# jskvrna/MonoSOWA

Measured on AMD Instinct MI355X. Metric: MonoDETR training img/s (KITTI 1280x384), higher is better.
Workload: dtype f32; 1 GPU; MonoDETR resnet50 KITTI 1280x384, fwd+criterion+bwd+AdamW step, per-GPU batch 16, synthetic images + random pseudo-labels; global_batch=16, per_gpu_batch=16, parallelism=dp1, accumulation_micro_steps=1, mixed_cameras=False, queries=550, tuned=True

## Files before the change

### include/monosowa_pointwise.h

```cpp
#ifndef MONOSOWA_POINTWISE_H_
#define MONOSOWA_POINTWISE_H_
#ifdef __cplusplus
extern "C" {
#endif

int mono_set_deterministic(int on);

int mono_bias_act_f32(float *y, const float *bias, const float *residual, long long rows, int C, int relu, void *stream);
int mono_bias_relu_maxpool_nhwc_f32(const float *y, const float *bias, float *out, int N, int H, int W, int C, void *stream);
int mono_conv1x1_tail_f32(const float *x, const float *b_in, const float *w, const float *b_out, const float *res, float *y,
                          long long M, int K, int N, void *stream);
int mono_conv1x1_tail_ds_f32(const float *x, const float *b_in, const float *w, const float *x0, const float *wd, const float *b_out,
                             float *y, long long M, int K, int N, void *stream);
int mono_conv1x1_head_f32(const float *x, const float *w, const float *b_out, float *y, long long M, int K, int N, void *stream);

int mono_relu_grad_f32(const float *grad_out, const float *y, float *grad_in, long long n, void *stream);
int mono_relu_grad_scale_f32(const float *grad_out, const float *y, const float *scale, float *grad_in, long long n, int C, void *stream);

int mono_bias_relu_mask_f32(float *y, const float *bias, const float *residual, unsigned char *mask, long long rows, int C,
                            void *stream);
int mono_relu_grad_mask_f32(const float *grad_a, const float *grad_b, const unsigned char *mask, float *grad_in, long long n,
                            void *stream);
int mono_relu_grad_mask3_f32(const float *grad_a, const float *grad_b, const float *grad_c, const unsigned char *mask, float *grad_in,
                             long long n, void *stream);
// ... 40 lines not shown
int mono_grad_guard_f32(const void *const *tables, const int *n_chunks, int n_groups, float max_norm, int skip_nonfinite,
                        double *partials, void *record, void *stream);
int mono_adamw_step_guarded_f32(const void *table, int n_chunks, double beta1, double beta2, double eps, double step_size,
                                const void *record, void *stream);

int mono_grad_accumulate_f32(const void *table, int n_chunks, void *stream);

int mono_ema_update_f32(const void *table, int n_chunks, float w, const void *record, void *stream);

int mono_step_stats_f32(const void *const *tables, const int *n_chunks, const int *const *groups, int n_tables, int n_groups,
                        const void *record, double *partials, double *out, void *stream);

long long mono_linear_wgrad_workspace(int R, int M, int N);
int mono_linear_wgrad_f32(const float *dy, long long ldy, const float *x, long long ldx, float *dw, float *db, float *ws, int R, int M,
                          int N, void *stream);

int mono_colsum_any_blocks(long long rows);
int mono_colsum_any_f32(const float *g, float *out, float *partials, long long rows, int C, void *stream);

int mono_sum_slices_f32(const float *x, float *out, int n, long long C, void *stream);

int mono_reduce_blocks(long long rows);

int mono_dropout_add_layernorm_bwd_f32(const float *gy, const float *s, const float *mean, const float *rstd,
                                       const float *gamma, float *gx, float *gz, float *ggamma_gbeta, float *partials,
                                       long long rows, int C, float p, unsigned long long seed, void *stream);

int mono_colsum_f32(const float *g, float *out, float *partials, long long rows, int C, void *stream);
int mono_colsum_strided_f32(const float *g, float *out, float *partials, int batch, long long rows, long long batch_stride,
                            int C, void *stream);
// ... 111 lines not shown
```

### monosowa_amd/csrc/pointwise.hip

```cpp
#include <hip/hip_runtime.h>

#include "relu_nan.h"
#include "groupnorm.hip"
#include "matched_losses.hip"
#include "ddn_loss.hip"
#include "head_tail.hip"
#include "lsap_device.hip"
#include "conv1x1_fused.hip"
#include "small_wgrad.hip"
#include <stdint.h>
#include <algorithm>

namespace mono {

template <bool RELU, bool RES>
__global__ __launch_bounds__(256) void bias_act_kernel(float *__restrict__ y, const float *__restrict__ bias,
                                                       const float *__restrict__ residual, long long n_vec, int c_vec) {
  const long long stride = (long long)gridDim.x * blockDim.x;
  for (long long i = (long long)blockIdx.x * blockDim.x + threadIdx.x; i < n_vec; i += stride) {
    float4 v = reinterpret_cast<float4 *>(y)[i];
    const float4 b = reinterpret_cast<const float4 *>(bias)[i % c_vec];
    v.x += b.x; v.y += b.y; v.z += b.z; v.w += b.w;
    if (RES) {
      const float4 r = reinterpret_cast<const float4 *>(residual)[i];
// ... 1081 lines not shown
  if (rows <= 0 || C <= 0 || C % 4 || C > 1024) return -2;
  hipStream_t st = (hipStream_t)stream_;
  if (rows <= mono::kColsumStripRows && C <= 384) {
    mono::colsum_strip_kernel<<<(C / 4 + 3) / 4, 1024, 0, st>>>(g, out, rows, C);
    return (int)hipGetLastError();
  }
  const int grid = mono_reduce_blocks(rows);
  const int rpb = (int)((rows + grid - 1) / grid + 63) / 64 * 64;
  if (C <= 256) mono::colsum_kernel<1><<<grid, 256, 0, st>>>(g, partials, rows, C, rpb, rows, 0);
  else if (C <= 512) mono::colsum_kernel<2><<<grid, 256, 0, st>>>(g, partials, rows, C, rpb, rows, 0);
  else mono::colsum_kernel<4><<<grid, 256, 0, st>>>(g, partials, rows, C, rpb, rows, 0);
  mono::partial_sum_kernel<<<(C / 4 + 63) / 64, 1024, 0, st>>>(partials, out, grid, C);
  return (int)hipGetLastError();
}

long long mono_linear_wgrad_workspace(int R, int M, int N) {
  if (R < 64 || R >= (1 << 24) || M <= 0 || N <= 0 || M % 64 || N % 64 || M > 4096 || N > 4096) return 0;
  return (long long)mono::linear_wgrad_splits(R, M, N) * ((long long)M * N + M);
}
int mono_linear_wgrad_f32(const float *dy, long long ldy, const float *x, long long ldx, float *dw, float *db, float *ws, int R, int M,
                          int N, void *stream_) {
  if (!dy || !x || !dw || !ws) return -1;
  if (!mono_linear_wgrad_workspace(R, M, N) || ldy < M || ldx < N || ldy % 4 || ldx % 4 || ((size_t)dy | (size_t)x | (size_t)dw | (size_t)ws) % 16 ||
      (db && (size_t)db % 16))
    return -2;
  hipStream_t st = (hipStream_t)stream_;
  const int S = mono::linear_wgrad_splits(R, M, N);
  const int rows_per_split = ((R + S - 1) / S + mono::kWgStageRows - 1) / mono::kWgStageRows * mono::kWgStageRows;
  const int tiles = (M / 64) * (N / 64);
  mono::linear_wgrad_partial_kernel<<<tiles * S, 256, 0, st>>>(dy, ldy, x, ldx, ws, R, M, N, S, rows_per_split);
  const long long MN = (long long)M * N;
  mono::linear_wgrad_reduce_kernel<<<(int)(((MN + M) / 4 + 255) / 256), 256, 0, st>>>(ws, dw, db, MN, M, S);
  return (int)hipGetLastError();
}

int mono_colsum_any_blocks(long long rows) {
  const long long b = (rows + 127) / 128;
  return (int)(b < 1 ? 1 : (b > 512 ? 512 : b));
}
int mono_colsum_any_f32(const float *g, float *out, float *partials, long long rows, int C, void *stream_) {
  if (!g || !out || !partials) return -1;
  if (rows <= 0 || C <= 0 || C > 1024) return -2;
  const int grid = mono_colsum_any_blocks(rows);
  const int rpb = (int)((rows + grid - 1) / grid);
  hipStream_t st = (hipStream_t)stream_;
  mono::colsum_scalar_kernel<<<grid, 256, 0, st>>>(g, partials, rows, C, rpb);
  mono::partial_sum_scalar_kernel<<<(C + 255) / 256, 256, 0, st>>>(partials, out, grid, C);
  return (int)hipGetLastError();
// ... 421 lines not shown
```

### monosowa_amd/csrc/small_wgrad.hip

```cpp
#pragma once
#include <hip/hip_runtime.h>

namespace mono {

typedef float wg_f32x16 __attribute__((ext_vector_type(16)));
#ifndef MONO_WGRAD_WORKGROUPS
#define MONO_WGRAD_WORKGROUPS 256
#endif
constexpr int kWgPairs = 8;
constexpr int kWgStageRows = 2 * kWgPairs;
constexpr int kWgSlots = 3;

inline int linear_wgrad_splits(int R, int M, int N) {
  const int tiles = (M / 64) * (N / 64);
  int S = ((MONO_WGRAD_WORKGROUPS + tiles - 1) / tiles + 7) / 8 * 8;
  while (S > 8 && R / S < 64) S -= 8;
  return S;
}

__global__ __launch_bounds__(256) void linear_wgrad_partial_kernel(const float *__restrict__ dy, long long ldy,
                                                                   const float *__restrict__ x, long long ldx, float *__restrict__ ws,
                                                                   int R, int M, int N, int S, int rows_per_split) {
  __shared__ float ring[kWgSlots][2][kWgStageRows * 64];
  const int s = blockIdx.x % S, tile = blockIdx.x / S;
  const int n_tiles = N / 64, tm = tile / n_tiles, tn = tile % n_tiles;
  const int lane = threadIdx.x & 63, wave = __builtin_amdgcn_readfirstlane(threadIdx.x >> 6), c = lane & 31, h = lane >> 5;
  const int wm = wave >> 1, wn = wave & 1;
  const int m0 = tm * 64 + wm * 32, n0 = tn * 64 + wn * 32;
  const int k_begin = s * rows_per_split, k_end = min(R, k_begin + rows_per_split);
  const int n_stages = k_end > k_begin ? (k_end - k_begin) / kWgStageRows : 0;
  wg_f32x16 acc0 = {0.f, 0.f, 0.f, 0.f, 0.f, 0.f, 0.f, 0.f, 0.f, 0.f, 0.f, 0.f, 0.f, 0.f, 0.f, 0.f}, acc1 = acc0;
  float bsum = 0.f;
  const int src_row = 4 * ((2 * wave) & 3) + 2 * (lane >> 5) + ((lane >> 3) & 1), src_col = 32 * ((lane >> 4) & 1) + 4 * (lane & 7);
  const float *gsrc = wave < 2 ? dy + (long long)(k_begin + src_row) * ldy + tm * 64 + src_col
                               : x + (long long)(k_begin + src_row) * ldx + tn * 64 + src_col;
  const long long g_ld = wave < 2 ? ldy : ldx;
  float *const lds_dst = &ring[0][wave >> 1][((2 * wave) & 3) * 256 + 4 * lane];
  constexpr int kSlotFloats = 2 * kWgStageRows * 64;
  const float *const al = &ring[0][0][wm * 64 + lane], *const bl = &ring[0][1][wn * 64 + lane];
  float4 g0a, g0b, g1a, g1b, g2a, g2b, g3a, g3b;
  float a0[kWgPairs], b0[kWgPairs], a1[kWgPairs], b1[kWgPairs];
#define WG_GLOAD(GA, GB, STAGE)                                                                                      \
  {                                                                                                                  \
    const float *p_ = gsrc + (long long)min((STAGE), n_stages - 1) * kWgStageRows * g_ld;              \
    GA = *reinterpret_cast<const float4 *>(p_); GB = *reinterpret_cast<const float4 *>(p_ + 4 * g_ld);               \
  }
#define WG_LWRITE(GA, GB, STAGE)                                                                                     \
  {                                                                                                                  \
    float *d_ = lds_dst + ((STAGE) % kWgSlots) * kSlotFloats;                                                        \
    *reinterpret_cast<float4 *>(d_) = GA; *reinterpret_cast<float4 *>(d_ + 256) = GB;                                \
  }
#define WG_STAGE(AC, BC, AN, BN, GA, GB, I)                                                                          \
  {                                                                                                                  \
    float *d_ = lds_dst + (((I) + 2) % kWgSlots) * kSlotFloats;                                                      \
    _Pragma("unroll") for (int u = 0; u < kWgPairs / 2; ++u) {                                                       \
      if (u & 1) acc1 = __builtin_amdgcn_mfma_f32_32x32x2f32(AC[u], BC[u], acc1, 0, 0, 0);                           \
      else acc0 = __builtin_amdgcn_mfma_f32_32x32x2f32(AC[u], BC[u], acc0, 0, 0, 0);                                 \
      bsum += AC[u];                                                                                                 \
      if (u < 2) {                           \
        __builtin_amdgcn_sched_barrier(0);                                                                           \
        *reinterpret_cast<float4 *>(d_ + 256 * u) = u ? GB : GA;                                                     \
        __builtin_amdgcn_sched_barrier(0);                                                                           \
      }                                                                                                              \
    }                                                                                                                \
    __builtin_amdgcn_sched_barrier(0);                                                                               \
    asm volatile("s_waitcnt lgkmcnt(0)" ::: "memory");                                                               \
    __builtin_amdgcn_s_barrier();                                                                                    \
    __builtin_amdgcn_sched_barrier(0);                                                                               \
    WG_GLOAD(GA, GB, (I) + 6)                                                                                        \
    __builtin_amdgcn_sched_barrier(0);                                                                               \
    const float *an_ = al + (((I) + 1) % kWgSlots) * kSlotFloats, *bn_ = bl + (((I) + 1) % kWgSlots) * kSlotFloats;  \
    _Pragma("unroll") for (int u = kWgPairs / 2; u < kWgPairs; ++u) {                                                \
      if (u & 1) acc1 = __builtin_amdgcn_mfma_f32_32x32x2f32(AC[u], BC[u], acc1, 0, 0, 0);                           \
      else acc0 = __builtin_amdgcn_mfma_f32_32x32x2f32(AC[u], BC[u], acc0, 0, 0, 0);                                 \
      bsum += AC[u];                                                                                                 \
      const int v = (u - kWgPairs / 2) * 2;                                                                          \
      AN[v] = an_[v * 128]; BN[v] = bn_[v * 128]; AN[v + 1] = an_[v * 128 + 128]; BN[v + 1] = bn_[v * 128 + 128];    \
      __builtin_amdgcn_sched_barrier(0);                                                                             \
    }                                                                                                                \
  }
  if (n_stages > 0) {
  WG_GLOAD(g0a, g0b, 0)
  WG_GLOAD(g1a, g1b, 1)
  WG_LWRITE(g0a, g0b, 0)
  WG_LWRITE(g1a, g1b, 1)
  WG_GLOAD(g0a, g0b, 2)
  WG_GLOAD(g1a, g1b, 3)
  WG_GLOAD(g2a, g2b, 4)
  WG_GLOAD(g3a, g3b, 5)
  __syncthreads();
// ... 15 lines not shown
#undef WG_GLOAD
#undef WG_LWRITE
  {
    const int k_tail = k_begin + n_stages * kWgStageRows;
    if (k_tail < k_end) {
      const float *ap = dy + (long long)(k_tail + h) * ldy + m0 + c, *bp = x + (long long)(k_tail + h) * ldx + n0 + c;
      float ta[kWgPairs], tb[kWgPairs];
#pragma unroll
      for (int u = 0; u < kWgPairs; ++u) {
        const bool live = k_tail + 2 * u + h < k_end;
        ta[u] = live ? ap[2 * u * ldy] : 0.f; tb[u] = live ? bp[2 * u * ldx] : 0.f;
      }
#pragma unroll
      for (int u = 0; u < kWgPairs; ++u) {
        acc0 = __builtin_amdgcn_mfma_f32_32x32x2f32(ta[u], tb[u], acc0, 0, 0, 0);
        bsum += ta[u];
      }
    }
  }
  float *wp = ws + (long long)s * ((long long)M * N + M);
#pragma unroll
  for (int v = 0; v < 16; ++v)
    wp[(long long)(m0 + 8 * (v >> 2) + 4 * h + (v & 3)) * N + n0 + c] = acc0[v] + acc1[v];
  if (tn == 0 && wn == 0) {
    const float t = bsum + __shfl_xor(bsum, 32);
    if (h == 0) wp[(long long)M * N + m0 + c] = t;
  }
}

__global__ __launch_bounds__(256) void linear_wgrad_reduce_kernel(const float *__restrict__ ws, float *__restrict__ dw, float *__restrict__ db,
                                                                  long long MN, int M, int S) {
  const long long i4 = (long long)blockIdx.x * 256 + threadIdx.x, stride4 = (MN + M) / 4;
  if (i4 >= stride4) return;
  const float4 *p = reinterpret_cast<const float4 *>(ws) + i4;
  float4 a = p[0];
#pragma unroll 4
  for (int s = 1; s < S; ++s) { const float4 b = p[s * stride4]; a.x += b.x; a.y += b.y; a.z += b.z; a.w += b.w; }
  if (i4 * 4 < MN) reinterpret_cast<float4 *>(dw)[i4] = a;
  else if (db) reinterpret_cast<float4 *>(db)[i4 - MN / 4] = a;
}

}
```

### monosowa_amd/flops.py

```python

_acc = None


def start():
    global _acc
    _acc = {}


def stop():
    global _acc
    out, _acc = _acc or {}, None
    return out


def add(kind, flops):
    if _acc is not None:
        _acc[kind] = _acc.get(kind, 0) + int(flops)


def attention_forward(B, H, Lq, Lk, d=32):
    add("attention_fwd", 2 * 2 * B * H * Lq * Lk * d)


def attention_backward(B, H, Lq, Lk, d=32):
    add("attention_bwd", 5 * 2 * B * H * Lq * Lk * d)


def conv1x1(M, K, N):
    add("conv1x1_fused", 2 * M * K * N)


def linear_wgrad(R, M, N):
    add("linear_wgrad", 2 * R * M * N)
```

### monosowa_amd/monodetr/depthaware_transformer.py

```python
import copy

import torch
import torch.nn.functional as F
from torch import nn
from torch.nn.init import constant_, normal_, xavier_uniform_

from .misc import inverse_sigmoid
from .. import MultiScaleDeformableAttention as _MSDA
from ..ms_deform_attn import MSDeformAttn
from .. import encoder_block
from ..flash_attn import mha_forward, mha_supported
from ..pointwise import dropout_add_layernorm, refine_reference, refine_reference_supported, relu_dropout
from ..token_linear import linear as fast_linear, token_linear


LEVEL_EMBED_IN_BLOCK = True
ENCODER_BLOCKS = True
MERGE_HEADS = False
MERGE_SA_PROJ = True
SELF_ATTN_HIP = True


class MLP(nn.Module):

    def __init__(self, input_dim, hidden_dim, output_dim, num_layers):
        super().__init__()
# ... 205 lines not shown
            q = fast_linear(x, self.sa_qcontent_proj.weight + self.sa_qpos_proj.weight, self.sa_qcontent_proj.bias + self.sa_qpos_proj.bias)
            k = fast_linear(x, self.sa_kcontent_proj.weight + self.sa_kpos_proj.weight, self.sa_kcontent_proj.bias + self.sa_kpos_proj.bias)
        else:
            q = self.sa_qcontent_proj(x) + self.sa_qpos_proj(x)
            k = self.sa_kcontent_proj(x) + self.sa_kpos_proj(x)
        return self._mha(mha, fold(q), fold(k), fold(v)).transpose(0, 1).reshape(B, Lq, C)

    @staticmethod
    def _mha(mha, q, k, v):
        if SELF_ATTN_HIP and mha_supported(mha, q, k, v):
            return mha_forward(mha, q, k, v)
        return mha(q, k, v, need_weights=False)[0]

    def forward(self, tgt, query_pos, reference_points, src, src_spatial_shapes, level_start_index,
                src_padding_mask, depth_pos_embed, mask_depth, value=None):
        tq = tgt.transpose(0, 1)
        if mha_supported(self.cross_attn_depth, tq, depth_pos_embed, depth_pos_embed, mask_depth):
            tgt2 = mha_forward(self.cross_attn_depth, tq, depth_pos_embed, depth_pos_embed, key_padding_mask=mask_depth).transpose(0, 1)
        else:
            tgt2 = self.cross_attn_depth(tq, depth_pos_embed, depth_pos_embed,
                                         key_padding_mask=mask_depth, need_weights=False)[0].transpose(0, 1)
        tgt = dropout_add_layernorm(tgt, tgt2, self.norm_depth, self.dropout_depth)
        tgt = dropout_add_layernorm(tgt, self._self_attention(tgt, query_pos), self.norm2, self.dropout2)
        tgt2 = self.cross_attn(_add_pos(tgt, query_pos), reference_points, src, src_spatial_shapes,
                               level_start_index, src_padding_mask, value=value)
        tgt = dropout_add_layernorm(tgt, tgt2, self.norm1, self.dropout1)
        ff = token_linear(relu_dropout(token_linear(tgt, self.linear1), self.dropout3), self.linear2)
        return dropout_add_layernorm(tgt, ff, self.norm3, self.dropout4)


# ... 167 lines not shown
```

### monosowa_amd/pointwise.py

```python
import ctypes
import os

import numpy as np
import torch

from . import flops
from ._lib import raw_stream, on_device, DeterministicSwitch, alert_not_deterministic

_PATH = os.path.join(os.path.dirname(os.path.abspath(__file__)), "lib", "libmonosowa_pointwise.so")
SYMBOLS = ("mono_bias_act_f32", "mono_bias_relu_maxpool_nhwc_f32", "mono_conv1x1_tail_f32", "mono_conv1x1_tail_ds_f32", "mono_conv1x1_head_f32", "mono_relu_grad_f32", "mono_relu_grad2_f32", "mono_relu_grad3_f32", "mono_bias_relu_mask_f32", "mono_relu_grad_mask_f32", "mono_affine_relu_mask_f32", "mono_affine_relu_grad_f32", "mono_dropout_add_layernorm_fwd_f32",
           "mono_dropout_add_layernorm_bwd_f32", "mono_groupnorm_nhwc_fwd_f32", "mono_groupnorm_nhwc_bwd_f32", "mono_groupnorm_blocks", "mono_colsum_f32", "mono_colsum_strided_f32", "mono_reduce_blocks", "mono_adamw_step_f32", "mono_adamw_step_guarded_f32", "mono_grad_guard_f32", "mono_relu_dropout_fwd_f32",
           "mono_relu_dropout_bwd_f32", "mono_matched_losses_fwd_f32", "mono_matched_losses_bwd_f32", "mono_ddn_loss_blocks",
           "mono_ddn_loss_fwd_f32", "mono_ddn_loss_bwd_f32", "mono_depth_expect_fwd_f32", "mono_depth_expect_bwd_f32", "mono_focal_fwd_f32", "mono_focal_bwd_f32", "mono_head_tail_fwd_f32", "mono_head_tail_bwd_f32", "mono_match_cost_f32", "mono_refine_reference_f32", "mono_relu_dropout_bwd_colsum_f32", "mono_sum_slices_f32", "mono_colsum_any_blocks", "mono_colsum_any_f32", "mono_relu_grad_mask3_f32", "mono_lsap_match_flat_f32",
           "mono_linear_wgrad_workspace", "mono_linear_wgrad_f32", "mono_colsum_levels_blocks", "mono_colsum_levels_f32", "mono_relu_grad_scale_f32",
           "mono_set_deterministic", "mono_groupnorm_stats_doubles", "mono_groupnorm_part_doubles", "mono_grad_accumulate_f32", "mono_ema_update_f32", "mono_step_stats_f32",
           "mono_label_audit_f32", "mono_matched_losses_weighted_fwd_f32", "mono_matched_losses_weighted_bwd_f32", "mono_focal_weighted_fwd_f32",
           "mono_focal_weighted_bwd_f32", "mono_ddn_loss_weighted_fwd_f32", "mono_ddn_loss_weighted_bwd_f32", "mono_focal_weighted_max_cells",
           "mono_ignore_flags_f32", "mono_focal_ignore_fwd_f32", "mono_focal_ignore_bwd_f32", "mono_focal_weighted_ignore_fwd_f32",
           "mono_focal_weighted_ignore_bwd_f32", "mono_ddn_loss_ignore_fwd_f32", "mono_ddn_loss_ignore_bwd_f32",
           "mono_ddn_loss_weighted_ignore_fwd_f32", "mono_ddn_loss_weighted_ignore_bwd_f32")
_lib = None


def load():
    global _lib
    if _lib is None:
        path = os.environ.get("MONOSOWA_POINTWISE_LIB", _PATH)
        if not os.path.exists(path):
            raise RuntimeError("HIP extension %s is missing: run `python -m monosowa_amd.build`" % path)
# ... 76 lines not shown
        lib.mono_step_stats_f32.argtypes = [P, P, P, I, I, P, P, P, P]
        lib.mono_label_audit_f32.restype = I
        lib.mono_label_audit_f32.argtypes = [P] * 13 + [I] * 7 + [P]
        lib.mono_colsum_strided_f32.restype = I
        lib.mono_colsum_strided_f32.argtypes = [P, P, P, I, LL, LL, I, P]
        lib.mono_colsum_levels_blocks.restype = I
        lib.mono_colsum_levels_blocks.argtypes = [I, LL, I, P]
        lib.mono_colsum_levels_f32.restype = I
        lib.mono_colsum_levels_f32.argtypes = [P, P, P, I, LL, I, I, P, I, P]
        lib.mono_colsum_f32.restype = I
        lib.mono_colsum_f32.argtypes = [P, P, P, LL, I, P]
        lib.mono_linear_wgrad_workspace.restype = LL
        lib.mono_linear_wgrad_workspace.argtypes = [I, I, I]
        lib.mono_linear_wgrad_f32.restype = I
        lib.mono_linear_wgrad_f32.argtypes = [P, LL, P, LL, P, P, P, I, I, I, P]
        lib.mono_ddn_loss_blocks.restype = I
        lib.mono_ddn_loss_blocks.argtypes = [I, I, I]
        lib.mono_ddn_loss_fwd_f32.restype = I
        lib.mono_ddn_loss_fwd_f32.argtypes = [P] * 5 + [I] * 5 + [LL] * 3 + [F] * 6 + [P]
        lib.mono_ddn_loss_bwd_f32.restype = I
        lib.mono_ddn_loss_bwd_f32.argtypes = [P] * 6 + [I] * 5 + [LL] * 3 + [F] * 6 + [P]
        lib.mono_depth_expect_fwd_f32.restype = I
        lib.mono_depth_expect_fwd_f32.argtypes = [P] * 3 + [I] * 4 + [LL] * 3 + [P]
        lib.mono_depth_expect_bwd_f32.restype = I
        lib.mono_depth_expect_bwd_f32.argtypes = [P] * 5 + [I] * 4 + [LL] * 3 + [P]
        lib.mono_match_cost_f32.restype = I
        lib.mono_match_cost_f32.argtypes = [P] * 6 + [I] * 5 + [F] * 4 + [P]
        lib.mono_focal_fwd_f32.restype = I
        lib.mono_focal_fwd_f32.argtypes = [P] * 5 + [I] * 5 + [F, F, P]
        lib.mono_focal_bwd_f32.restype = I
# ... 552 lines not shown
        raise ValueError("linear_wgrad: unsupported operands %s %s" % (tuple(g2.shape), tuple(x2.shape)))
    R, M = g2.shape
    N = x2.shape[1]
    flops.linear_wgrad(R, M, N)
    ws = torch.empty(_wgrad_workspace(R, M, N), dtype=torch.float32, device=g2.device)
    out = torch.empty(M * N + M, dtype=torch.float32, device=g2.device)
    p = out.data_ptr()
    with on_device(g2.device):
        code = load().mono_linear_wgrad_f32(g2.data_ptr(), g2.stride(0), x2.data_ptr(), x2.stride(0), p, p + 4 * M * N if with_bias else None,
                                            ws.data_ptr(), R, M, N, raw_stream())
    if code:
        raise RuntimeError("mono_linear_wgrad_f32 failed with code %d" % code)
    return out[:M * N].view(M, N), (out[M * N:] if with_bias else None)


def colsum(g2):
    rows, C = (g2.shape if g2.dim() == 2 else (0, 0))
    if rows > 0 and C % 4 == 0 and C <= COLSUM_MAX_C and g2.is_cuda and g2.dtype == torch.float32 and g2.is_contiguous() \
            and g2.data_ptr() % 16 == 0:
        lib = load()
        buf = torch.empty((lib.mono_reduce_blocks(rows) + 1) * C, dtype=torch.float32, device=g2.device)
        p0 = buf.data_ptr()
        if g2.device.index == torch.cuda.current_device():
            code = lib.mono_colsum_f32(g2.data_ptr(), p0, p0 + 4 * C, rows, C, raw_stream())
        else:
            with on_device(g2.device):
                code = lib.mono_colsum_f32(g2.data_ptr(), p0, p0 + 4 * C, rows, C, raw_stream())
        if code:
            raise RuntimeError("mono_colsum_f32 failed with code %d" % code)
        return buf[:C]
# ... 913 lines not shown
```

Before: 243.9 img/s.

## Add fused decoder-layer autograd blocks with grouped linear weight-gradient kernel

Adds a grouped weight-gradient API that packs up to eight linear wgrad problems into one partial and one reduce launch, using a per-block lookup table. The bias column sum is now accumulated only in the waves that write it. A new decoder_block module replaces the MonoDETR decoder layer's depth attention, self-attention and FFN with custom autograd Functions that call flash attention, fused layernorm and the grouped wgrad directly. The aim is to cut launch count and autograd overhead in the decoder backward, at the cost of much more custom code and workspace bookkeeping per call.

```diff
diff --git a/include/monosowa_pointwise.h b/include/monosowa_pointwise.h
--- a/include/monosowa_pointwise.h
+++ b/include/monosowa_pointwise.h
@@ -78,6 +78,15 @@
 long long mono_linear_wgrad_workspace(int R, int M, int N);
 int mono_linear_wgrad_f32(const float *dy, long long ldy, const float *x, long long ldx, float *dw, float *db, float *ws, int R, int M,
                           int N, void *stream);
+
+typedef struct {
+  const float *dy; long long ldy;
+  const float *x; long long ldx;
+  float *dw; float *db;
+  int R, M, N;
+} mono_wgrad_problem;
+long long mono_linear_wgrad_group_workspace(const mono_wgrad_problem *problems, int n);
+int mono_linear_wgrad_group_f32(const mono_wgrad_problem *problems, int n, float *ws, void *stream);
 
 int mono_colsum_any_blocks(long long rows);
 int mono_colsum_any_f32(const float *g, float *out, float *partials, long long rows, int C, void *stream);
diff --git a/monosowa_amd/csrc/pointwise.hip b/monosowa_amd/csrc/pointwise.hip
--- a/monosowa_amd/csrc/pointwise.hip
+++ b/monosowa_amd/csrc/pointwise.hip
@@ -1119,24 +1119,72 @@
   return (int)hipGetLastError();
 }
 
+static bool wgrad_shape_served(int R, int M, int N) {
+  return !(R < 64 || R >= (1 << 24) || M <= 0 || N <= 0 || M % 64 || N % 64 || M > 4096 || N > 4096);
+}
 long long mono_linear_wgrad_workspace(int R, int M, int N) {
-  if (R < 64 || R >= (1 << 24) || M <= 0 || N <= 0 || M % 64 || N % 64 || M > 4096 || N > 4096) return 0;
+  if (!wgrad_shape_served(R, M, N)) return 0;
   return (long long)mono::linear_wgrad_splits(R, M, N) * ((long long)M * N + M);
+}
+
+struct mono_wgrad_problem {
+  const float *dy; long long ldy;
+  const float *x; long long ldx;
+  float *dw, *db;
+  int R, M, N;
+};
+static long long wgrad_group_plan(const mono_wgrad_problem *p, int n, mono::WgGroup *g, int *partial_grid, int *reduce_grid) {
+  if (!p || n < 1 || n > mono::kWgMaxGroup) return 0;
+  long long group_tiles = 0;
+  for (int i = 0; i < n; ++i) {
+    if (!wgrad_shape_served(p[i].R, p[i].M, p[i].N)) return 0;
+    group_tiles += (p[i].M / 64) * (p[i].N / 64);
+  }
+  long long ws = 0, wgs = 0, reds = 0;
+  for (int i = 0; i < mono::kWgMaxGroup; ++i) {
+    mono::WgProblem &q = g->p[i];
+    if (i >= n) { q = mono::WgProblem{}; q.wg_end = q.red_end = INT32_MAX; continue; }
+    const int R = p[i].R, M = p[i].M, N = p[i].N;
+    const int S = mono::linear_wgrad_group_splits(R, (int)std::min<long long>(group_tiles, 1 << 20), n);
+    q.dy = p[i].dy; q.x = p[i].x; q.dw = p[i].dw; q.db = p[i].db; q.ldy = p[i].ldy; q.ldx = p[i].ldx;
+    q.R = R; q.M = M; q.N = N; q.S = S; q.ws_off = ws;
+    q.rows_per_split = ((R + S - 1) / S + mono::kWgStageRows - 1) / mono::kWgStageRows * mono::kWgStageRows;
+    const long long image = (long long)M * N + M;
+    ws += S * image;
+    wgs += (long long)(M / 64) * (N / 64) * S;
+    reds += (image / 4 + 255) / 256;
+    if (wgs >= INT32_MAX || reds >= INT32_MAX) return 0;
+    q.wg_end = (int)wgs; q.red_end = (int)reds;
+  }
+  *partial_grid = (int)wgs; *reduce_grid = (int)reds;
+  return ws;
+}
+long long mono_linear_wgrad_group_workspace(const mono_wgrad_problem *p, int n) {
+  mono::WgGroup g;
+  int a, b;
+  return wgrad_group_plan(p, n, &g, &a, &b);
+}
+int mono_linear_wgrad_group_f32(const mono_wgrad_problem *p, int n, float *ws, void *stream_) {
+  if (!p || !ws) return -1;
+  if (n < 1 || n > mono::kWgMaxGroup) return -2;
+  for (int i = 0; i < n; ++i) {
+    if (!p[i].dy || !p[i].x || !p[i].dw) return -1;
+    if (p[i].M <= 0 || p[i].N <= 0 || p[i].ldy < p[i].M || p[i].ldx < p[i].N || p[i].ldy % 4 || p[i].ldx % 4 ||
+        ((size_t)p[i].dy | (size_t)p[i].x | (size_t)p[i].dw | (size_t)p[i].db | (size_t)ws) % 16)
+      return -2;
+  }
+  mono::WgGroup g;
+  int partial_grid, reduce_grid;
+  if (!wgrad_group_plan(p, n, &g, &partial_grid, &reduce_grid)) return -2;
+  hipStream_t st = (hipStream_t)stream_;
+  mono::linear_wgrad_partial_kernel<<<partial_grid, 256, 0, st>>>(g, ws);
+  mono::linear_wgrad_reduce_kernel<<<reduce_grid, 256, 0, st>>>(g, ws);
+  return (int)hipGetLastError();
 }
 int mono_linear_wgrad_f32(const float *dy, long long ldy, const float *x, long long ldx, float *dw, float *db, float *ws, int R, int M,
                           int N, void *stream_) {
-  if (!dy || !x || !dw || !ws) return -1;
-  if (!mono_linear_wgrad_workspace(R, M, N) || ldy < M || ldx < N || ldy % 4 || ldx % 4 || ((size_t)dy | (size_t)x | (size_t)dw | (size_t)ws) % 16 ||
-      (db && (size_t)db % 16))
-    return -2;
-  hipStream_t st = (hipStream_t)stream_;
-  const int S = mono::linear_wgrad_splits(R, M, N);
-  const int rows_per_split = ((R + S - 1) / S + mono::kWgStageRows - 1) / mono::kWgStageRows * mono::kWgStageRows;
-  const int tiles = (M / 64) * (N / 64);
-  mono::linear_wgrad_partial_kernel<<<tiles * S, 256, 0, st>>>(dy, ldy, x, ldx, ws, R, M, N, S, rows_per_split);
-  const long long MN = (long long)M * N;
-  mono::linear_wgrad_reduce_kernel<<<(int)(((MN + M) / 4 + 255) / 256), 256, 0, st>>>(ws, dw, db, MN, M, S);
-  return (int)hipGetLastError();
+  const mono_wgrad_problem p = {dy, ldy, x, ldx, dw, db, R, M, N};
+  return mono_linear_wgrad_group_f32(&p, 1, ws, stream_);
 }
 
 int mono_colsum_any_blocks(long long rows) {
diff --git a/monosowa_amd/csrc/small_wgrad.hip b/monosowa_amd/csrc/small_wgrad.hip
--- a/monosowa_amd/csrc/small_wgrad.hip
+++ b/monosowa_amd/csrc/small_wgrad.hip
@@ -18,19 +18,41 @@
   return S;
 }
 
-__global__ __launch_bounds__(256) void linear_wgrad_partial_kernel(const float *__restrict__ dy, long long ldy,
-                                                                   const float *__restrict__ x, long long ldx, float *__restrict__ ws,
-                                                                   int R, int M, int N, int S, int rows_per_split) {
-  __shared__ float ring[kWgSlots][2][kWgStageRows * 64];
-  const int s = blockIdx.x % S, tile = blockIdx.x / S;
-  const int n_tiles = N / 64, tm = tile / n_tiles, tn = tile % n_tiles;
-  const int lane = threadIdx.x & 63, wave = __builtin_amdgcn_readfirstlane(threadIdx.x >> 6), c = lane & 31, h = lane >> 5;
+#ifndef MONO_WGRAD_GROUP_WORKGROUPS
+#define MONO_WGRAD_GROUP_WORKGROUPS (2 * MONO_WGRAD_WORKGROUPS)
+#endif
+inline int linear_wgrad_group_splits(int R, int group_tiles, int n_problems) {
+  const int target = n_problems > 1 ? MONO_WGRAD_GROUP_WORKGROUPS : MONO_WGRAD_WORKGROUPS;
+  int S = ((target + group_tiles - 1) / group_tiles + 7) / 8 * 8;
+  while (S > 8 && R / S < 64) S -= 8;
+  return S;
+}
+
+constexpr int kWgMaxGroup = 8;
+struct WgProblem {
+  const float *dy, *x;
+  float *dw, *db;
+  long long ldy, ldx, ws_off;
+  int R, M, N, S, rows_per_split;
+  int wg_end, red_end;
+};
+struct WgGroup { WgProblem p[kWgMaxGroup]; };
+
+__device__ __forceinline__ int wgrad_problem_of(const WgGroup &g, int bid, bool reduce) {
+  int pi = 0;
+#pragma unroll
+  for (int i = 0; i < kWgMaxGroup - 1; ++i) pi += bid >= (reduce ? g.p[i].red_end : g.p[i].wg_end) ? 1 : 0;
+  return pi;
+}
+
+template <bool kBias>
+__device__ __forceinline__ void wgrad_rows(const float *__restrict__ dy, long long ldy, const float *__restrict__ x, long long ldx,
+                                           float (*ring)[2][kWgStageRows * 64], int k_begin, int k_end, int tm, int tn, int wave, int lane,
+                                           wg_f32x16 &acc0, wg_f32x16 &acc1, float &bsum) {
+  const int c = lane & 31, h = lane >> 5;
   const int wm = wave >> 1, wn = wave & 1;
   const int m0 = tm * 64 + wm * 32, n0 = tn * 64 + wn * 32;
-  const int k_begin = s * rows_per_split, k_end = min(R, k_begin + rows_per_split);
   const int n_stages = k_end > k_begin ? (k_end - k_begin) / kWgStageRows : 0;
-  wg_f32x16 acc0 = {0.f, 0.f, 0.f, 0.f, 0.f, 0.f, 0.f, 0.f, 0.f, 0.f, 0.f, 0.f, 0.f, 0.f, 0.f, 0.f}, acc1 = acc0;
-  float bsum = 0.f;
   const int src_row = 4 * ((2 * wave) & 3) + 2 * (lane >> 5) + ((lane >> 3) & 1), src_col = 32 * ((lane >> 4) & 1) + 4 * (lane & 7);
   const float *gsrc = wave < 2 ? dy + (long long)(k_begin + src_row) * ldy + tm * 64 + src_col
                                : x + (long long)(k_begin + src_row) * ldx + tn * 64 + src_col;
@@ -56,7 +78,7 @@
     _Pragma("unroll") for (int u = 0; u < kWgPairs / 2; ++u) {                                                       \
       if (u & 1) acc1 = __builtin_amdgcn_mfma_f32_32x32x2f32(AC[u], BC[u], acc1, 0, 0, 0);                           \
       else acc0 = __builtin_amdgcn_mfma_f32_32x32x2f32(AC[u], BC[u], acc0, 0, 0, 0);                                 \
-      bsum += AC[u];                                                                                                 \
+      if (kBias) bsum += AC[u];                                                                                      \
       if (u < 2) {                           \
         __builtin_amdgcn_sched_barrier(0);                                                                           \
         *reinterpret_cast<float4 *>(d_ + 256 * u) = u ? GB : GA;                                                     \
@@ -73,7 +95,7 @@
     _Pragma("unroll") for (int u = kWgPairs / 2; u < kWgPairs; ++u) {                                                \
       if (u & 1) acc1 = __builtin_amdgcn_mfma_f32_32x32x2f32(AC[u], BC[u], acc1, 0, 0, 0);                           \
       else acc0 = __builtin_amdgcn_mfma_f32_32x32x2f32(AC[u], BC[u], acc0, 0, 0, 0);                                 \
-      bsum += AC[u];                                                                                                 \
+      if (kBias) bsum += AC[u];                                                                                      \
       const int v = (u - kWgPairs / 2) * 2;                                                                          \
       AN[v] = an_[v * 128]; BN[v] = bn_[v * 128]; AN[v + 1] = an_[v * 128 + 128]; BN[v + 1] = bn_[v * 128 + 128];    \
       __builtin_amdgcn_sched_barrier(0);                                                                             \
@@ -119,23 +141,48 @@
 #pragma unroll
       for (int u = 0; u < kWgPairs; ++u) {
         acc0 = __builtin_amdgcn_mfma_f32_32x32x2f32(ta[u], tb[u], acc0, 0, 0, 0);
-        bsum += ta[u];
+        if (kBias) bsum += ta[u];
       }
     }
   }
-  float *wp = ws + (long long)s * ((long long)M * N + M);
+}
+
+__global__ __launch_bounds__(256) void linear_wgrad_partial_kernel(const WgGroup g, float *__restrict__ ws) {
+  __shared__ float ring[kWgSlots][2][kWgStageRows * 64];
+  const int pi = wgrad_problem_of(g, blockIdx.x, false);
+  const WgProblem &pr = g.p[pi];
+  const int bid = blockIdx.x - (pi ? g.p[pi - 1].wg_end : 0);
+  const int R = pr.R, M = pr.M, N = pr.N, S = pr.S, rows_per_split = pr.rows_per_split;
+  const int s = bid % S, tile = bid / S;
+  const int n_tiles = N / 64, tm = tile / n_tiles, tn = tile % n_tiles;
+  const int lane = threadIdx.x & 63, wave = __builtin_amdgcn_readfirstlane(threadIdx.x >> 6), c = lane & 31, h = lane >> 5;
+  const int wm = wave >> 1, wn = wave & 1;
+  const int m0 = tm * 64 + wm * 32, n0 = tn * 64 + wn * 32;
+  const int k_begin = s * rows_per_split, k_end = min(R, k_begin + rows_per_split);
+  wg_f32x16 acc0 = {0.f, 0.f, 0.f, 0.f, 0.f, 0.f, 0.f, 0.f, 0.f, 0.f, 0.f, 0.f, 0.f, 0.f, 0.f, 0.f}, acc1 = acc0;
+  float bsum = 0.f;
+  const bool bias_wave = tn == 0 && wn == 0 && pr.db != nullptr;
+  if (bias_wave) wgrad_rows<true>(pr.dy, pr.ldy, pr.x, pr.ldx, ring, k_begin, k_end, tm, tn, wave, lane, acc0, acc1, bsum);
+  else wgrad_rows<false>(pr.dy, pr.ldy, pr.x, pr.ldx, ring, k_begin, k_end, tm, tn, wave, lane, acc0, acc1, bsum);
+  float *wp = ws + pr.ws_off + (long long)s * ((long long)M * N + M);
 #pragma unroll
   for (int v = 0; v < 16; ++v)
     wp[(long long)(m0 + 8 * (v >> 2) + 4 * h + (v & 3)) * N + n0 + c] = acc0[v] + acc1[v];
-  if (tn == 0 && wn == 0) {
+  if (bias_wave) {
     const float t = bsum + __shfl_xor(bsum, 32);
     if (h == 0) wp[(long long)M * N + m0 + c] = t;
   }
 }
 
-__global__ __launch_bounds__(256) void linear_wgrad_reduce_kernel(const float *__restrict__ ws, float *__restrict__ dw, float *__restrict__ db,
-                                                                  long long MN, int M, int S) {
-  const long long i4 = (long long)blockIdx.x * 256 + threadIdx.x, stride4 = (MN + M) / 4;
+__global__ __launch_bounds__(256) void linear_wgrad_reduce_kernel(const WgGroup g, const float *__restrict__ ws_all) {
+  const int pi = wgrad_problem_of(g, blockIdx.x, true);
+  const WgProblem &pr = g.p[pi];
+  const int bid = blockIdx.x - (pi ? g.p[pi - 1].red_end : 0);
+  const int M = pr.M, S = pr.S;
+  const long long MN = (long long)M * pr.N;
+  const float *ws = ws_all + pr.ws_off;
+  float *dw = pr.dw, *db = pr.db;
+  const long long i4 = (long long)bid * 256 + threadIdx.x, stride4 = (MN + M) / 4;
   if (i4 >= stride4) return;
   const float4 *p = reinterpret_cast<const float4 *>(ws) + i4;
   float4 a = p[0];
diff --git a/monosowa_amd/decoder_block.py b/monosowa_amd/decoder_block.py
--- /dev/null
+++ b/monosowa_amd/decoder_block.py
@@ -0,0 +1,259 @@
+import math
+import os
+
+import torch
+import torch.nn.functional as F
+
+from . import flash_attn, flops, token_linear
+from . import pointwise as pw
+from ._lib import on_device, raw_stream
+
+ENABLED = os.environ.get("MONOSOWA_DECODER_BLOCKS", "1") != "0"
+GROUPED = {"depth": True, "self": True, "ffn": True}
+_SCALE = 1.0 / math.sqrt(32.0)
+
+
+def _wgrads(kind, pairs, outs=None):
+    if GROUPED[kind]:
+        return pw.linear_wgrad_group(pairs, True, outs)
+    res = []
+    for i, (g2, x2, with_bias) in enumerate(pairs):
+        gw, gb = pw.linear_wgrad(g2, x2, with_bias, True)
+        if outs is not None and outs[i] is not None:
+            outs[i][0].copy_(gw)
+            if with_bias:
+                outs[i][1].copy_(gb)
+            gw, gb = outs[i][0], (outs[i][1] if with_bias else None)
+        res.append((gw, gb))
+    return res
+
+
+def _attn_fwd(q, k, v, p, seed, mask):
+    B, H, Lq, _ = q.shape
+    o = flash_attn._like_heads(q)
+    lse = torch.empty((B * H, Lq), dtype=torch.float32, device=q.device)
+    mp, mask = flash_attn._mask_ptr(mask, B, k.size(2))
+    bits = flash_attn.keep_bits_like(q, k, p) if flash_attn.SAVE_KEEP_BITS else None
+    flops.attention_forward(B, H, Lq, k.size(2))
+    st = flash_attn._strides
+    with on_device(q.device):
+        code = flash_attn.load().mono_attn_forward_keep_f32(q.data_ptr(), k.data_ptr(), v.data_ptr(), mp, bits.data_ptr() if bits is not None else 0,
+                                                            o.data_ptr(), lse.data_ptr(), B, H, Lq, k.size(2), 32, st(q), st(k), st(v), st(o),
+                                                            _SCALE, float(p), seed, raw_stream())
+    if code:
+        raise RuntimeError("mono_attn_forward_keep_f32 failed with code %d" % code)
+    return o, lse, bits
+
+
+def _attn_bwd(q, k, v, o, lse, dout, dq, dk, dv, p, seed, mask, bits):
+    B, H, Lq, _ = q.shape
+    Lk = k.size(2)
+    delta = torch.empty((B * H, Lq), dtype=torch.float32, device=q.device)
+    assert dout.stride() == o.stride()
+    mp, mask = flash_attn._mask_ptr(mask, B, Lk)
+    flops.attention_backward(B, H, Lq, Lk)
+    st = flash_attn._strides
+    with on_device(q.device):
+        code = flash_attn.load().mono_attn_backward_keep_f32(q.data_ptr(), k.data_ptr(), v.data_ptr(), mp, bits.data_ptr() if bits is not None else 0,
+                                                             o.data_ptr(), lse.data_ptr(), dout.data_ptr(), dq.data_ptr(), dk.data_ptr(),
+                                                             dv.data_ptr(), delta.data_ptr(), B, H, Lq, Lk, 32, st(q), st(k), st(v), st(o),
+                                                             st(dq), st(dk), st(dv), _SCALE, float(p), seed, raw_stream())
+    if code:
+        raise RuntimeError("mono_attn_backward_keep_f32 failed with code %d" % code)
+
+
+def _heads(t, batch_major, H):
+    t4 = t.unflatten(-1, (H, 32))
+    return t4.permute(0, 2, 1, 3) if batch_major else t4.permute(1, 2, 0, 3)
+
+
+class _DepthAttnBlock(torch.autograd.Function):
+
+    @staticmethod
+    def forward(ctx, tgt, depth, mask, w_in, b_in, w_out, b_out, gamma, beta, H, p_attn, p_res, eps):
+        B, Lq, E = tgt.shape
+        ctx.bm = not depth.is_contiguous() and depth.transpose(0, 1).is_contiguous()
+        kb = depth.transpose(0, 1) if ctx.bm else depth.contiguous()
+        q = F.linear(tgt, w_in[:E], b_in[:E])
+        kv = F.linear(kb, w_in[E:], b_in[E:])
+        seed = flash_attn._next_seed() if p_attn > 0 else 0
+        o, lse, bits = _attn_fwd(_heads(q, True, H), _heads(kv[..., :E], ctx.bm, H), _heads(kv[..., E:], ctx.bm, H), p_attn, seed, mask)
+        o = o.permute(0, 2, 1, 3).reshape(B, Lq, E)
+        z = F.linear(o, w_out, b_out)
+        y, s, mean, rstd, ln_seed = pw.ln_forward(tgt, z, gamma, beta, p_res, eps)
+        ctx.save_for_backward(tgt, kb, q, kv, o, lse, s, mean, rstd, w_in, w_out, gamma)
+        ctx.H, ctx.p_attn, ctx.seed, ctx.mask, ctx.bits, ctx.p_res, ctx.ln_seed = H, p_attn, seed, mask, bits, p_res, ln_seed
+        return y
+
+    @staticmethod
+    def backward(ctx, gy):
+        tgt, kb, q, kv, o, lse, s, mean, rstd, w_in, w_out, gamma = ctx.saved_tensors
+        B, Lq, E = tgt.shape
+        H, bm = ctx.H, ctx.bm
+        gx, gz, ggamma, gbeta, gb_out = pw.ln_backward(gy, s, mean, rstd, gamma, ctx.p_res, ctx.ln_seed, with_gz_sum=True)
+        gz2 = gz.view(-1, E)
+        go = (gz2 @ w_out).view(B, Lq, E)
+        dq, dkv = torch.empty_like(q), torch.empty_like(kv)
+        _attn_bwd(_heads(q, True, H), _heads(kv[..., :E], bm, H), _heads(kv[..., E:], bm, H), _heads(o, True, H), lse, _heads(go, True, H),
+                  _heads(dq, True, H), _heads(dkv[..., :E], bm, H), _heads(dkv[..., E:], bm, H), ctx.p_attn, ctx.seed, ctx.mask, ctx.bits)
+        dq2, dkv2 = dq.view(-1, E), dkv.view(-1, 2 * E)
+        gx.view(-1, E).addmm_(dq2, w_in[:E])
+        g_depth = None
+        if ctx.needs_input_grad[1]:
+            g_depth = (dkv2 @ w_in[E:]).view(kb.shape)
+            if bm:
+                g_depth = g_depth.transpose(0, 1)
+        gw_in, gb_in = torch.empty_like(w_in), torch.empty(3 * E, dtype=torch.float32, device=tgt.device)
+        (gw_out, _), _, _ = _wgrads("depth", [(gz2, o.view(-1, E), False), (dq2, tgt.view(-1, E), True), (dkv2, kb.reshape(-1, E), True)],
+                                    [None, (gw_in[:E], gb_in[:E]), (gw_in[E:], gb_in[E:])])
+        return gx, g_depth, None, gw_in, gb_in, gw_out, gb_out, ggamma, gbeta, None, None, None, None
+
+
+class _SelfAttnBlock(torch.autograd.Function):
+
+    @staticmethod
+    def forward(ctx, tgt, query_pos, wqc, bqc, wqp, bqp, wkc, bkc, wkp, bkp, w_in, b_in, w_out, b_out, gamma, beta, H, n, p_attn, p_res, eps):
+        B, Lq, E = tgt.shape
+        x = tgt + query_pos
+        wq, bq, wk, bk = wqc + wqp, bqc + bqp, wkc + wkp, bkc + bkp
+        q1, k1 = F.linear(x, wq, bq), F.linear(x, wk, bk)
+        q2 = F.linear(q1, w_in[:E], b_in[:E])
+        k2 = F.linear(k1, w_in[E:2 * E], b_in[E:2 * E])
+        v2 = F.linear(tgt, w_in[2 * E:], b_in[2 * E:])
+        seed = flash_attn._next_seed() if p_attn > 0 else 0
+        fold = lambda t: _heads(t.view(-1, n, E), True, H)
+        o, lse, bits = _attn_fwd(fold(q2), fold(k2), fold(v2), p_attn, seed, None)
+        o = o.permute(0, 2, 1, 3).reshape(B, Lq, E)
+        z = F.linear(o, w_out, b_out)
+        y, s, mean, rstd, ln_seed = pw.ln_forward(tgt, z, gamma, beta, p_res, eps)
+        ctx.save_for_backward(tgt, x, q1, k1, q2, k2, v2, o, lse, s, mean, rstd, wq, wk, w_in, w_out, gamma)
+        ctx.H, ctx.n, ctx.p_attn, ctx.seed, ctx.bits, ctx.p_res, ctx.ln_seed = H, n, p_attn, seed, bits, p_res, ln_seed
+        return y
+
+    @staticmethod
+    def backward(ctx, gy):
+        tgt, x, q1, k1, q2, k2, v2, o, lse, s, mean, rstd, wq, wk, w_in, w_out, gamma = ctx.saved_tensors
+        B, Lq, E = tgt.shape
+        H, n = ctx.H, ctx.n
+        gx, gz, ggamma, gbeta, gb_out = pw.ln_backward(gy, s, mean, rstd, gamma, ctx.p_res, ctx.ln_seed, with_gz_sum=True)
+        gz2 = gz.view(-1, E)
+        go = (gz2 @ w_out).view(B, Lq, E)
+        dq, dk, dv = torch.empty_like(q2), torch.empty_like(k2), torch.empty_like(v2)
+        fold = lambda t: _heads(t.view(-1, n, E), True, H)
+        _attn_bwd(fold(q2), fold(k2), fold(v2), fold(o), lse, fold(go), fold(dq), fold(dk), fold(dv), ctx.p_attn, ctx.seed, None, ctx.bits)
+        dq2, dk2, dv2, gx2 = dq.view(-1, E), dk.view(-1, E), dv.view(-1, E), gx.view(-1, E)
+        gx2.addmm_(dv2, w_in[2 * E:])
+        gq1, gk1 = dq2 @ w_in[:E], dk2 @ w_in[E:2 * E]
+        gpos = gq1 @ wq
+        gpos.addmm_(gk1, wk)
+        gx2 += gpos
+        gw_in, gb_in = torch.empty_like(w_in), torch.empty(3 * E, dtype=torch.float32, device=tgt.device)
+        x2 = x.view(-1, E)
+        res = _wgrads("self", [(gz2, o.view(-1, E), False), (dq2, q1.view(-1, E), True), (dk2, k1.view(-1, E), True), (dv2, tgt.view(-1, E), True),
+                               (gq1, x2, True), (gk1, x2, True)],
+                      [None, (gw_in[:E], gb_in[:E]), (gw_in[E:2 * E], gb_in[E:2 * E]), (gw_in[2 * E:], gb_in[2 * E:]), None, None])
+        gw_out, (gwq, gbq), (gwk, gbk) = res[0][0], res[4], res[5]
+        return (gx, gpos.view(B, Lq, E), gwq, gbq, gwq, gbq, gwk, gbk, gwk, gbk, gw_in, gb_in, gw_out, gb_out, ggamma, gbeta,
+                None, None, None, None, None)
+
+
+class _FFNBlock(torch.autograd.Function):
+
+    @staticmethod
+    def forward(ctx, x, w1, b1, w2, b2, gamma, beta, p_hidden, p_res, eps):
+        h = F.linear(x, w1, b1)
+        hd = pw.relu_dropout_forward(h, p_hidden) if p_hidden > 0 else torch.relu_(h)
+        f = F.linear(hd, w2, b2)
+        y, s, mean, rstd, seed = pw.ln_forward(x, f, gamma, beta, p_res, eps)
+        ctx.save_for_backward(x, hd, s, mean, rstd, w1, w2, gamma)
+        ctx.p_hidden, ctx.p_res, ctx.seed = p_hidden, p_res, seed
+        return y
+
+    @staticmethod
+    def backward(ctx, gy):
+        x, hd, s, mean, rstd, w1, w2, gamma = ctx.saved_tensors
+        C, Hd = x.shape[-1], hd.shape[-1]
+        gx, gf, ggamma, gbeta, gb2 = pw.ln_backward(gy, s, mean, rstd, gamma, ctx.p_res, ctx.seed, with_gz_sum=True)
+        gf2 = gf.view(-1, C)
+        ghd = (gf2 @ w2).view_as(hd)
+        gh = pw.relu_dropout_backward(ghd, hd, ctx.p_hidden) if ctx.p_hidden > 0 else ghd * (hd > 0)
+        gh2 = gh.view(-1, Hd)
+        gx.view(-1, C).addmm_(gh2, w1)
+        (gw2, _), (gw1, gb1) = _wgrads("ffn", [(gf2, hd.view(-1, Hd), False), (gh2, x.view(-1, C), True)])
+        return gx, gw1, gb1, gw2, gb2, ggamma, gbeta, None, None, None
+
+
+def _norm_ok(norm, drop):
+    return tuple(norm.normalized_shape) == (256,) and norm.elementwise_affine and norm.bias is not None and drop.p < 1.0
+
+
+def _mha_ok(mha):
+    return (mha.embed_dim == 256 and mha.num_heads == 8 and not mha.batch_first and mha._qkv_same_embed_dim and mha.in_proj_bias is not None
+            and mha.bias_k is None and not mha.add_zero_attn and mha.out_proj.bias is not None and 0.0 <= mha.dropout < 1.0)
+
+
+def _served(R, M, N):
+    return pw._wgrad_workspace(R, M, N) > 0
+
+
+def _trainable(layer):
+    ok = layer.__dict__.get("_decoder_block_params")
+    if ok is None:
+        ok = layer.__dict__["_decoder_block_params"] = [p for name, p in layer.named_parameters()
+                                                        if not name.startswith(("sa_v_proj", "cross_attn.value_proj"))]
+    return all(p.requires_grad and p.dtype == torch.float32 for p in ok)
+
+
+def supported(layer, tgt, query_pos, reference_points, spatial_shapes, level_start_index, padding_mask, depth_tokens, mask_depth):
+    from .monodetr import depthaware_transformer as dt
+    from . import ms_deform_attn as msda_mod, ms_deform_attn_func as msda_func
+    if not (ENABLED and tgt.is_cuda and tgt.dtype == torch.float32 and torch.is_grad_enabled() and layer.training and tgt.dim() == 3
+            and tgt.shape[-1] == 256 and query_pos is not None and query_pos.dtype == torch.float32 and query_pos.shape == tgt.shape
+            and depth_tokens.dim() == 3 and depth_tokens.dtype == torch.float32 and depth_tokens.shape[1:] == (tgt.shape[0], 256)):
+        return False
+    B, Lq, _ = tgt.shape
+    rows, rows_k = B * Lq, depth_tokens.shape[0] * B
+    G, n = layer.group_num, layer.group_size
+    if not (token_linear.FAST_LINEAR and token_linear.SMALL_WGRAD_KERNEL and token_linear.FAST_MIN_ROWS <= rows < token_linear.MIN_TOKENS
+            and rows_k < token_linear.MIN_TOKENS and rows >= pw.LN_MIN_ROWS and Lq == G * n and dt.SELF_ATTN_HIP and dt.MERGE_SA_PROJ):
+        return False
+    Hd = layer.linear1.out_features
+    if not (_served(rows, 256, 256) and _served(rows_k, 512, 256) and _served(rows, 384, 256) and _served(rows, Hd, 256) and _served(rows, 256, Hd)
+            and layer.linear2.in_features == Hd and layer.linear1.in_features == 256):
+        return False
+    if not (_mha_ok(layer.cross_attn_depth) and _mha_ok(layer.self_attn) and B * 8 <= 65535 and B * G * 8 <= 65535
+            and flash_attn.mask_supported(mask_depth, B, depth_tokens.shape[0], tgt.device)
+            and all(_norm_ok(nm, d) for nm, d in ((layer.norm_depth, layer.dropout_depth), (layer.norm2, layer.dropout2),
+                                                  (layer.norm1, layer.dropout1), (layer.norm3, layer.dropout4)))):
+        return False
+    p3 = layer.dropout3.p
+    if not (p3 == 0.0 or (0.0 < p3 < 1.0 and rows * Hd >= pw.RELU_DROPOUT_MIN_NUMEL)):
+        return False
+    ca = layer.cross_attn
+    geom = getattr(spatial_shapes, "_msda_host_geometry", None)
+    if not (ca.fuse_prologue and msda_mod.MERGED_PROJ and ca.n_levels == 4 and ca.n_points == 4 and ca.n_heads == 8 and ca.d_model == 256
+            and (not reference_points.requires_grad or reference_points.shape[-1] == 2) and reference_points.shape[-1] in (2, 6)
+            and reference_points.dtype == torch.float32 and geom is not None and (padding_mask is None or msda_mod.MASK_IN_KERNEL)
+            and msda_func.MSDeformAttnFunction.__module__ == msda_func.__name__):
+        return False
+    return _trainable(layer)
+
+
+def decoder_layer(layer, tgt, query_pos, reference_points, src, spatial_shapes, level_start_index, padding_mask, depth_tokens, mask_depth,
+                  value=None):
+    if not supported(layer, tgt, query_pos, reference_points, spatial_shapes, level_start_index, padding_mask, depth_tokens, mask_depth):
+        return None
+    if not tgt.is_contiguous():
+        tgt = tgt.contiguous()
+    mha = layer.cross_attn_depth
+    tgt = _DepthAttnBlock.apply(tgt, depth_tokens, mask_depth, mha.in_proj_weight, mha.in_proj_bias, mha.out_proj.weight, mha.out_proj.bias,
+                                layer.norm_depth.weight, layer.norm_depth.bias, 8, mha.dropout, layer.dropout_depth.p, layer.norm_depth.eps)
+    mha = layer.self_attn
+    qc, qp, kc, kp = layer.sa_qcontent_proj, layer.sa_qpos_proj, layer.sa_kcontent_proj, layer.sa_kpos_proj
+    tgt = _SelfAttnBlock.apply(tgt, query_pos, qc.weight, qc.bias, qp.weight, qp.bias, kc.weight, kc.bias, kp.weight, kp.bias,
+                               mha.in_proj_weight, mha.in_proj_bias, mha.out_proj.weight, mha.out_proj.bias, layer.norm2.weight,
+                               layer.norm2.bias, 8, layer.group_size, mha.dropout, layer.dropout2.p, layer.norm2.eps)
+    tgt2 = layer.cross_attn(tgt + query_pos, reference_points, src, spatial_shapes, level_start_index, padding_mask, value=value)
+    tgt = pw.dropout_add_layernorm(tgt, tgt2, layer.norm1, layer.dropout1)
+    return _FFNBlock.apply(tgt, layer.linear1.weight, layer.linear1.bias, layer.linear2.weight, layer.linear2.bias, layer.norm3.weight,
+                           layer.norm3.bias, layer.dropout3.p, layer.dropout4.p, layer.norm3.eps)
diff --git a/monosowa_amd/flops.py b/monosowa_amd/flops.py
--- a/monosowa_amd/flops.py
+++ b/monosowa_amd/flops.py
@@ -32,3 +32,7 @@
 
 def linear_wgrad(R, M, N):
     add("linear_wgrad", 2 * R * M * N)
+
+
+def linear_wgrad_group(shapes):
+    add("linear_wgrad", sum(2 * R * M * N for R, M, N in shapes))
diff --git a/monosowa_amd/monodetr/depthaware_transformer.py b/monosowa_amd/monodetr/depthaware_transformer.py
--- a/monosowa_amd/monodetr/depthaware_transformer.py
+++ b/monosowa_amd/monodetr/depthaware_transformer.py
@@ -9,7 +9,9 @@
 from .. import MultiScaleDeformableAttention as _MSDA
 from ..ms_deform_attn import MSDeformAttn
 from .. import encoder_block
+from .. import decoder_block
 from ..flash_attn import mha_forward, mha_supported
+from .. import pointwise as _pointwise
 from ..pointwise import dropout_add_layernorm, refine_reference, refine_reference_supported, relu_dropout
 from ..token_linear import linear as fast_linear, token_linear
 
@@ -245,6 +247,11 @@
 
     def forward(self, tgt, query_pos, reference_points, src, src_spatial_shapes, level_start_index,
                 src_padding_mask, depth_pos_embed, mask_depth, value=None):
+        if decoder_block.ENABLED and dropout_add_layernorm is _pointwise.dropout_add_layernorm and relu_dropout is _pointwise.relu_dropout:
+            out = decoder_block.decoder_layer(self, tgt, query_pos, reference_points, src, src_spatial_shapes, level_start_index,
+                                              src_padding_mask, depth_pos_embed, mask_depth, value)
+            if out is not None:
+                return out
         tq = tgt.transpose(0, 1)
         if mha_supported(self.cross_attn_depth, tq, depth_pos_embed, depth_pos_embed, mask_depth):
             tgt2 = mha_forward(self.cross_attn_depth, tq, depth_pos_embed, depth_pos_embed, key_padding_mask=mask_depth).transpose(0, 1)
diff --git a/monosowa_amd/pointwise.py b/monosowa_amd/pointwise.py
--- a/monosowa_amd/pointwise.py
+++ b/monosowa_amd/pointwise.py
@@ -12,7 +12,7 @@
            "mono_dropout_add_layernorm_bwd_f32", "mono_groupnorm_nhwc_fwd_f32", "mono_groupnorm_nhwc_bwd_f32", "mono_groupnorm_blocks", "mono_colsum_f32", "mono_colsum_strided_f32", "mono_reduce_blocks", "mono_adamw_step_f32", "mono_adamw_step_guarded_f32", "mono_grad_guard_f32", "mono_relu_dropout_fwd_f32",
            "mono_relu_dropout_bwd_f32", "mono_matched_losses_fwd_f32", "mono_matched_losses_bwd_f32", "mono_ddn_loss_blocks",
            "mono_ddn_loss_fwd_f32", "mono_ddn_loss_bwd_f32", "mono_depth_expect_fwd_f32", "mono_depth_expect_bwd_f32", "mono_focal_fwd_f32", "mono_focal_bwd_f32", "mono_head_tail_fwd_f32", "mono_head_tail_bwd_f32", "mono_match_cost_f32", "mono_refine_reference_f32", "mono_relu_dropout_bwd_colsum_f32", "mono_sum_slices_f32", "mono_colsum_any_blocks", "mono_colsum_any_f32", "mono_relu_grad_mask3_f32", "mono_lsap_match_flat_f32",
-           "mono_linear_wgrad_workspace", "mono_linear_wgrad_f32", "mono_colsum_levels_blocks", "mono_colsum_levels_f32", "mono_relu_grad_scale_f32",
+           "mono_linear_wgrad_workspace", "mono_linear_wgrad_f32", "mono_linear_wgrad_group_workspace", "mono_linear_wgrad_group_f32", "mono_colsum_levels_blocks", "mono_colsum_levels_f32", "mono_relu_grad_scale_f32",
            "mono_set_deterministic", "mono_groupnorm_stats_doubles", "mono_groupnorm_part_doubles", "mono_grad_accumulate_f32", "mono_ema_update_f32", "mono_step_stats_f32",
            "mono_label_audit_f32", "mono_matched_losses_weighted_fwd_f32", "mono_matched_losses_weighted_bwd_f32", "mono_focal_weighted_fwd_f32",
            "mono_focal_weighted_bwd_f32", "mono_ddn_loss_weighted_fwd_f32", "mono_ddn_loss_weighted_bwd_f32", "mono_focal_weighted_max_cells",
@@ -119,6 +119,10 @@
         lib.mono_linear_wgrad_workspace.argtypes = [I, I, I]
         lib.mono_linear_wgrad_f32.restype = I
         lib.mono_linear_wgrad_f32.argtypes = [P, LL, P, LL, P, P, P, I, I, I, P]
+        lib.mono_linear_wgrad_group_workspace.restype = LL
+        lib.mono_linear_wgrad_group_workspace.argtypes = [P, I]
+        lib.mono_linear_wgrad_group_f32.restype = I
+        lib.mono_linear_wgrad_group_f32.argtypes = [P, I, P, P]
         lib.mono_ddn_loss_blocks.restype = I
         lib.mono_ddn_loss_blocks.argtypes = [I, I, I]
         lib.mono_ddn_loss_fwd_f32.restype = I
@@ -701,6 +705,59 @@
     return out[:M * N].view(M, N), (out[M * N:] if with_bias else None)
 
 
+class _WgradProblem(ctypes.Structure):
+    _fields_ = [("dy", ctypes.c_void_p), ("ldy", ctypes.c_longlong), ("x", ctypes.c_void_p), ("ldx", ctypes.c_longlong),
+                ("dw", ctypes.c_void_p), ("db", ctypes.c_void_p), ("R", ctypes.c_int), ("M", ctypes.c_int), ("N", ctypes.c_int)]
+
+
+WGRAD_GROUP_MAX = 8
+_WGRAD_GROUP_WS = {}
+
+
+def linear_wgrad_group(pairs, checked=False, outs=None):
+    n = len(pairs)
+    if not 1 <= n <= WGRAD_GROUP_MAX:
+        raise ValueError("linear_wgrad_group: 1 .. %d problems, got %d" % (WGRAD_GROUP_MAX, n))
+    if not checked:
+        for g2, x2, _ in pairs:
+            if not linear_wgrad_applies(g2, x2) or g2.device != pairs[0][0].device:
+                raise ValueError("linear_wgrad_group: unsupported operands %s %s" % (tuple(g2.shape), tuple(x2.shape)))
+    device = pairs[0][0].device
+    shapes = tuple((g2.shape[0], g2.shape[1], x2.shape[1]) for g2, x2, _ in pairs)
+    flops.linear_wgrad_group(shapes)
+    table = (_WgradProblem * n)()
+    given = outs if outs is not None else [None] * n
+    total = sum(M * N + M for (R, M, N), o in zip(shapes, given) if o is None)
+    out = torch.empty(total, dtype=torch.float32, device=device) if total else None
+    p, off, results = (out.data_ptr() if total else 0), 0, []
+    for t, (g2, x2, with_bias), (R, M, N), o in zip(table, pairs, shapes, given):
+        t.dy, t.ldy, t.x, t.ldx, t.R, t.M, t.N = g2.data_ptr(), g2.stride(0), x2.data_ptr(), x2.stride(0), R, M, N
+        if o is None:
+            t.dw, t.db = p + 4 * off, (p + 4 * (off + M * N) if with_bias else None)
+            results.append((out[off:off + M * N].view(M, N), out[off + M * N:off + M * N + M] if with_bias else None))
+            off += M * N + M
+        else:
+            dw, db = o
+            if not (dw.is_contiguous() and dw.dtype == torch.float32 and dw.device == device and dw.numel() == M * N
+                    and dw.data_ptr() % 16 == 0) or (with_bias and (db is None or not db.is_contiguous() or db.dtype != torch.float32
+                                                                     or db.device != device or db.numel() != M or db.data_ptr() % 16)):
+                raise ValueError("linear_wgrad_group: unsuitable output tensors for problem %s" % ((R, M, N),))
+            t.dw, t.db = dw.data_ptr(), (db.data_ptr() if with_bias else None)
+            results.append((dw, db if with_bias else None))
+    lib = load()
+    n_ws = _WGRAD_GROUP_WS.get(shapes)
+    if n_ws is None:
+        n_ws = _WGRAD_GROUP_WS[shapes] = lib.mono_linear_wgrad_group_workspace(ctypes.addressof(table), n)
+    if n_ws <= 0:
+        raise ValueError("linear_wgrad_group: shapes not served: %s" % (shapes,))
+    ws = torch.empty(n_ws, dtype=torch.float32, device=device)
+    with on_device(device):
+        code = lib.mono_linear_wgrad_group_f32(ctypes.addressof(table), n, ws.data_ptr(), raw_stream())
+    if code:
+        raise RuntimeError("mono_linear_wgrad_group_f32 failed with code %d" % code)
+    return results
+
+
 def colsum(g2):
     rows, C = (g2.shape if g2.dim() == 2 else (0, 0))
     if rows > 0 and C % 4 == 0 and C <= COLSUM_MAX_C and g2.is_cuda and g2.dtype == torch.float32 and g2.is_contiguous() \
```

After: 247.7 img/s, median of 6. Within noise of the previous version (+1.6%).
